# TheoCoombes/ClipCap

Measured on AMD Instinct MI355X. Metric: train samples/sec (512-d prefix, 40-tok caption), higher is better.
Workload: dtype bf16; 1 GPU; BASELINE configs[1]: TransformerMapper(8L,P=L=10,H=8)+frozen GPT-2-small; per_gpu_batch=256, global_batch=256, encoder_dim=512, train_language_model=False, parallelism=dp1

## Files before the change

clipcap_amd/csrc/attention.hip:

```cpp
#include "kernels.h"

namespace CC_NS {

__device__ __forceinline__ void load_head_rows(float* dst, int hdp, const act_t* src, size_t ld, int S, int hd) {
    const int c8n = hd >> 3;
    for (int idx = threadIdx.x; idx < S * c8n; idx += blockDim.x) {
        const int r = idx / c8n, c = idx % c8n;
        float f[8];
        act_ld8(src + (size_t)r * ld + c * 8, f);
        float* d = dst + r * hdp + c * 8;
        *reinterpret_cast<float4*>(d) = make_float4(f[0], f[1], f[2], f[3]);
        *reinterpret_cast<float4*>(d + 4) = make_float4(f[4], f[5], f[6], f[7]);
    }
}

template <auto Kernel, class... Args>
static void attn_launch(dim3 grid, dim3 block, size_t sh, hipStream_t st, const Args&... args) {
    if (sh > 64 * 1024) (void)hipFuncSetAttribute((const void*)Kernel, hipFuncAttributeMaxDynamicSharedMemorySize, (int)sh);
    hipLaunchKernelGGL(Kernel, grid, block, sh, st, args...);
}
#define ATTN_LADDER(LAUNCH) { if (drop.thresh) { LAUNCH(true, true); } else if (causal) { LAUNCH(true, false); } else { LAUNCH(false, false); } }

__device__ __forceinline__ unsigned attn_drop_idx(int b, int H, int h, int S, int q, int k) { return ((unsigned)(b * H + h) * S + q) * S + k; }
template <bool CAUSAL>
// ... 579 lines not shown
        }
        float mx = -INFINITY;
#pragma unroll
        for (int r = 0; r < 16; r++) {
            const int kr = kb * 32 + c_row(r, half);
            const bool ok = kr < S && (!CAUSAL || kr <= q);
            s[r] = ok ? s[r] * scale : -INFINITY;
            mx = fmaxf(mx, s[r]);
        }
        mx = fmaxf(mx, __shfl_xor(mx, 32, 64));
        const float m_new = fmaxf(m, mx);
        const float alpha = (m == -INFINITY) ? 0.f : __expf(m - m_new);
        float p[16], ps = 0.f;
#pragma unroll
        for (int r = 0; r < 16; r++) {
            p[r] = (m_new == -INFINITY) ? 0.f : __expf(s[r] - m_new);
            ps += p[r];
        }
        ps += __shfl_xor(ps, 32, 64);
        l = l * alpha + ps;
        m = m_new;
#pragma unroll
        for (int nb = 0; nb < NB; nb++)
#pragma unroll
            for (int r = 0; r < 16; r++) o[nb][r] *= alpha;
        if (DROP) {
            const unsigned rowbase = attn_drop_idx(b, H, h, S, min(q, S - 1), 0);
#pragma unroll
            for (int r = 0; r < 16; r++) p[r] *= drop_mul(drop, rowbase + min(kb * 32 + c_row(r, half), S - 1));
        }
        op16x8 pf[2];
#pragma unroll
        for (int t = 0; t < 2; t++) pf[t] = pack_frag(p + t * 8);
#pragma unroll
        for (int t = 0; t < 2; t++)
#pragma unroll
            for (int nb = 0; nb < NB; nb++) o[nb] = CC_MFMA_32x32x16(frag_tr<HD>(vs, nb, t, lane), pf[t], o[nb]);
#pragma unroll
        for (int kk = 0; kk < KK; kk++) kq[kk] = kn[kk];
#pragma unroll
        for (int c = 0; c < HD / 16; c++) vq[c] = vn[c];
    }
    if (q < S) {
        const float inv = l > 0.f ? 1.f / l : 0.f;
        op16_t* orow = out + ((size_t)b * S + q) * D + h * HD;
        store_acc_row<NB, true>(orow, o, half, inv);
        if (half == 0 && lse_out) lse_out[((size_t)b * H + h) * S + q] = m + __logf(l);
    }
}

template <int HD>
static int attn_fwd_mfma_launch(const op16_t* qkv, int B, int S, int H, bool causal, op16_t* out, float* lse, hipStream_t st, Drop drop) {
    const int items = B * H * ((S + 31) / 32);
    const float scale = 1.0f / sqrtf((float)HD);
    if (drop.thresh && !causal) return CC_ERR_SHAPE;
#define CC_L(C, DR) attn_launch<k_attn_fwd_mfma<HD, C, DR>>(dim3((items + 3) / 4), dim3(256), 0, st, qkv, B, S, H, scale, out, lse, drop)
    ATTN_LADDER(CC_L)
#undef CC_L
    return hipGetLastError() == hipSuccess ? CC_OK : CC_ERR_LAUNCH;
}


template <int HD, bool CAUSAL, bool DROP = false>
__global__ __launch_bounds__(256, HD == 64 ? 2 : 1) void k_attn_bwd_dkv(const op16_t* __restrict__ qkv, const op16_t* __restrict__ dout,
                                                      const float* __restrict__ lse, const float* __restrict__ delta, int B, int S, int H,
                                                      float scale, op16_t* __restrict__ dqkv, Drop drop = Drop()) {
    constexpr int KK = HD / 16, NB = HD / 32;
    __shared__ __attribute__((aligned(16))) op16_t qsm[4][32 * AttLd<HD>::v];
    __shared__ __attribute__((aligned(16))) op16_t dsm[4][32 * AttLd<HD>::v];
    __shared__ __attribute__((aligned(16))) float ldsm[4][64];
    const int lane = threadIdx.x & 63, wave = threadIdx.x >> 6;
    const int nblk = (S + 31) >> 5;
    const int item = blockIdx.x * 4 + wave;
    if (item >= B * H * nblk) return;
    const int j = item % nblk, h = (item / nblk) % H, b = item / (nblk * H);
    const int D = H * HD;
    const size_t rs = (size_t)3 * D;
    const op16_t* base = qkv + (size_t)b * S * rs + h * HD;
    const op16_t* dbase = dout + (size_t)b * S * D + h * HD;
    const float* lrow = lse + ((size_t)b * H + h) * S;
    const float* drow = delta + ((size_t)b * H + h) * S;
    const int half = lane >> 5, key = j * 32 + (lane & 31);
    op16x8 kf[KK], vf[KK];
#pragma unroll
    for (int kk = 0; kk < KK; kk++) {
        kf[kk] = load_frag(base + D + (size_t)min(key, S - 1) * rs + kk * 16 + half * 8, key < S);
        vf[kk] = load_frag(base + 2 * D + (size_t)min(key, S - 1) * rs + kk * 16 + half * 8, key < S);
    }
    f32x16 dk[NB], dv[NB];
#pragma unroll
    for (int nb = 0; nb < NB; nb++)
#pragma unroll
        for (int r = 0; r < 16; r++) { dk[nb][r] = 0.f; dv[nb][r] = 0.f; }
    const int i0 = CAUSAL ? j : 0;
    op16x8 qf[KK], df[KK];
    {
        const int qa = i0 * 32 + (lane & 31);
#pragma unroll
        for (int kk = 0; kk < KK; kk++) {
            qf[kk] = load_frag(base + (size_t)min(qa, S - 1) * rs + kk * 16 + half * 8, qa < S);
            df[kk] = load_frag(dbase + (size_t)min(qa, S - 1) * D + kk * 16 + half * 8, qa < S);
        }
    }
    for (int i = i0; i < nblk; i++) {
        op16x8 qn[KK], dn[KK];
        {
            const int qa = (i + 1) * 32 + (lane & 31);
#pragma unroll
            for (int kk = 0; kk < KK; kk++) {
                qn[kk] = load_frag(base + (size_t)min(qa, S - 1) * rs + kk * 16 + half * 8, qa < S);
                dn[kk] = load_frag(dbase + (size_t)min(qa, S - 1) * D + kk * 16 + half * 8, qa < S);
            }
        }
        f32x16 s, dp;
#pragma unroll
        for (int r = 0; r < 16; r++) { s[r] = 0.f; dp[r] = 0.f; }
#pragma unroll
        for (int kk = 0; kk < KK; kk++) {
            s = CC_MFMA_32x32x16(qf[kk], kf[kk], s);
            dp = CC_MFMA_32x32x16(df[kk], vf[kk], dp);
            *reinterpret_cast<op16x8*>(qsm[wave] + (lane & 31) * AttLd<HD>::v + kk * 16 + half * 8) = qf[kk];
            *reinterpret_cast<op16x8*>(dsm[wave] + (lane & 31) * AttLd<HD>::v + kk * 16 + half * 8) = df[kk];
        }
        {
            const int qq = min(i * 32 + (lane & 31), S - 1);
            ldsm[wave][lane] = half ? drow[qq] : lrow[qq];
        }
        float lq[16], dq_[16];
#pragma unroll
        for (int g4 = 0; g4 < 4; g4++) {
            const float4 a = *reinterpret_cast<const float4*>(&ldsm[wave][4 * half + 8 * g4]);
            const float4 b = *reinterpret_cast<const float4*>(&ldsm[wave][32 + 4 * half + 8 * g4]);
            lq[g4 * 4 + 0] = a.x; lq[g4 * 4 + 1] = a.y; lq[g4 * 4 + 2] = a.z; lq[g4 * 4 + 3] = a.w;
            dq_[g4 * 4 + 0] = b.x; dq_[g4 * 4 + 1] = b.y; dq_[g4 * 4 + 2] = b.z; dq_[g4 * 4 + 3] = b.w;
        }
        float p[16], ds[16];
#pragma unroll
        for (int r = 0; r < 16; r++) {
            const int qr = i * 32 + c_row(r, half);
            const bool ok = attn_live<CAUSAL>(qr, key, S);
            p[r] = ok ? __expf(s[r] * scale - lq[r]) : 0.f;
            if (DROP) {
                const float mk = drop_mul(drop, attn_drop_idx(b, H, h, S, min(qr, S - 1), min(key, S - 1)));
                ds[r] = p[r] * (mk * dp[r] - dq_[r]) * scale;
                p[r] *= mk;
            } else {
                ds[r] = p[r] * (dp[r] - dq_[r]) * scale;
            }
        }
        const op16x8 pf[2] = {pack_frag(p), pack_frag(p + 8)};
        const op16x8 dsf[2] = {pack_frag(ds), pack_frag(ds + 8)};
#pragma unroll
        for (int t = 0; t < 2; t++)
#pragma unroll
            for (int nb = 0; nb < NB; nb++) {
                dv[nb] = CC_MFMA_32x32x16(frag_tr<HD>(dsm[wave], nb, t, lane), pf[t], dv[nb]);
                dk[nb] = CC_MFMA_32x32x16(frag_tr<HD>(qsm[wave], nb, t, lane), dsf[t], dk[nb]);
            }
#pragma unroll
        for (int kk = 0; kk < KK; kk++) { qf[kk] = qn[kk]; df[kk] = dn[kk]; }
    }
    if (key < S) {
        op16_t* orow = dqkv + ((size_t)b * S + key) * rs + h * HD;
#pragma unroll
        for (int nb = 0; nb < NB; nb++)
#pragma unroll
            for (int g = 0; g < 4; g++) {
                const int d0 = nb * 32 + 8 * g + 4 * half;
                *reinterpret_cast<uint2*>(orow + D + d0) =
                    make_uint2(pack2op(dk[nb][g * 4 + 0], dk[nb][g * 4 + 1]), pack2op(dk[nb][g * 4 + 2], dk[nb][g * 4 + 3]));
                *reinterpret_cast<uint2*>(orow + 2 * D + d0) =
                    make_uint2(pack2op(dv[nb][g * 4 + 0], dv[nb][g * 4 + 1]), pack2op(dv[nb][g * 4 + 2], dv[nb][g * 4 + 3]));
            }
    }
}

template <int HD, bool CAUSAL, bool DROP = false>
__global__ __launch_bounds__(256, HD == 64 ? 3 : (HD == 96 ? 2 : 1)) void k_attn_bwd_dq(const op16_t* __restrict__ qkv, const op16_t* __restrict__ dout, const op16_t* __restrict__ o,
                                                     const float* __restrict__ lse, float* __restrict__ delta, int B, int S, int H,
                                                     float scale, op16_t* __restrict__ dqkv, Drop drop = Drop()) {
    constexpr int KK = HD / 16, NB = HD / 32;
    __shared__ __attribute__((aligned(16))) op16_t ksm[4][32 * AttLd<HD>::v];
    const int lane = threadIdx.x & 63, wave = threadIdx.x >> 6;
    const int nblk = (S + 31) >> 5;
    const int item = blockIdx.x * 4 + wave;
    if (item >= B * H * nblk) return;
    const int i = item % nblk, h = (item / nblk) % H, b = item / (nblk * H);
    const int D = H * HD;
    const size_t rs = (size_t)3 * D;
    const op16_t* base = qkv + (size_t)b * S * rs + h * HD;
    const op16_t* dbase = dout + (size_t)b * S * D + h * HD;
    const int half = lane >> 5, q = i * 32 + (lane & 31);
    const float my_lse = q < S ? lse[((size_t)b * H + h) * S + q] : 0.f;
    op16x8 qf[KK], dof[KK];
    float my_delta = 0.f;
#pragma unroll
    for (int kk = 0; kk < KK; kk++) {
        qf[kk] = load_frag(base + (size_t)min(q, S - 1) * rs + kk * 16 + half * 8, q < S);
        dof[kk] = load_frag(dbase + (size_t)min(q, S - 1) * D + kk * 16 + half * 8, q < S);
        const op16x8 of = load_frag(o + ((size_t)b * S + min(q, S - 1)) * D + h * HD + kk * 16 + half * 8, q < S);
        float x[8], y[8];
        unpack8(__builtin_bit_cast(uint4, dof[kk]), x);
        unpack8(__builtin_bit_cast(uint4, of), y);
#pragma unroll
        for (int e = 0; e < 8; e++) my_delta += x[e] * y[e];
    }
    my_delta += __shfl_xor(my_delta, 32, 64);
    if (half == 0 && q < S) delta[((size_t)b * H + h) * S + q] = my_delta;
    f32x16 dq[NB];
#pragma unroll
    for (int nb = 0; nb < NB; nb++)
#pragma unroll
        for (int r = 0; r < 16; r++) dq[nb][r] = 0.f;
    const int jend = CAUSAL ? i + 1 : nblk;
    op16x8 kf[KK], vf[KK];
    {
        const int key = lane & 31;
#pragma unroll
        for (int kk = 0; kk < KK; kk++) {
            kf[kk] = load_frag(base + D + (size_t)min(key, S - 1) * rs + kk * 16 + half * 8, key < S);
            vf[kk] = load_frag(base + 2 * D + (size_t)min(key, S - 1) * rs + kk * 16 + half * 8, key < S);
        }
    }
    for (int j = 0; j < jend; j++) {
        op16x8 kn[KK], vn[KK];
        {
            const int key = (j + 1) * 32 + (lane & 31);
#pragma unroll
            for (int kk = 0; kk < KK; kk++) {
                kn[kk] = load_frag(base + D + (size_t)min(key, S - 1) * rs + kk * 16 + half * 8, key < S);
                vn[kk] = load_frag(base + 2 * D + (size_t)min(key, S - 1) * rs + kk * 16 + half * 8, key < S);
            }
        }
        f32x16 st, dpt;
#pragma unroll
        for (int r = 0; r < 16; r++) { st[r] = 0.f; dpt[r] = 0.f; }
#pragma unroll
        for (int kk = 0; kk < KK; kk++) {
            st = CC_MFMA_32x32x16(kf[kk], qf[kk], st);
            dpt = CC_MFMA_32x32x16(vf[kk], dof[kk], dpt);
            *reinterpret_cast<op16x8*>(ksm[wave] + (lane & 31) * AttLd<HD>::v + kk * 16 + half * 8) = kf[kk];
        }
        float ds[16];
#pragma unroll
        for (int r = 0; r < 16; r++) {
            const int kr = j * 32 + c_row(r, half);
            const bool ok = kr < S && q < S && (!CAUSAL || kr <= q);
            const float p = ok ? __expf(st[r] * scale - my_lse) : 0.f;
            const float mk = DROP ? drop_mul(drop, attn_drop_idx(b, H, h, S, min(q, S - 1), min(kr, S - 1))) : 1.0f;
            ds[r] = p * (mk * dpt[r] - my_delta) * scale;
        }
        const op16x8 dsf[2] = {pack_frag(ds), pack_frag(ds + 8)};
#pragma unroll
        for (int t = 0; t < 2; t++)
#pragma unroll
            for (int nb = 0; nb < NB; nb++)
                dq[nb] = CC_MFMA_32x32x16(frag_tr<HD>(ksm[wave], nb, t, lane), dsf[t], dq[nb]);
#pragma unroll
        for (int kk = 0; kk < KK; kk++) { kf[kk] = kn[kk]; vf[kk] = vn[kk]; }
    }
    if (q < S) {
        op16_t* orow = dqkv + ((size_t)b * S + q) * rs + h * HD;
        store_acc_row<NB>(orow, dq, half);
    }
}

#ifndef CC_ATTN_FUSED_OCC
#define CC_ATTN_FUSED_OCC 2
#endif
template <int LD, int ROWS = 32>
__device__ __forceinline__ op16x8 frag_tr_ld(const op16_t* blk, int nb, int t, int lane) {
    typedef __attribute__((ext_vector_type(4))) short s16x4_t;
    typedef __attribute__((address_space(3))) s16x4_t* lp_t;
    const int half = lane >> 5, j = lane & 15, dsub = (lane >> 4) & 1;
    const int r0 = 16 * t + 4 * half + (j >> 2);
    const op16_t* col = blk + nb * 32 + 16 * dsub + 4 * (j & 3);
    const op16_t* p = col + (ROWS < 32 ? min(r0, ROWS - 1) : r0) * LD;
    const op16_t* ph = col + (ROWS < 32 ? min(r0 + 8, ROWS - 1) : r0 + 8) * LD;
    const s16x4_t lo = __builtin_amdgcn_ds_read_tr16_b64_v4i16((lp_t)p);
    const s16x4_t hi = __builtin_amdgcn_ds_read_tr16_b64_v4i16((lp_t)ph);
    typedef __attribute__((ext_vector_type(8))) short s16x8_t;
    const s16x8_t v = {lo[0], lo[1], lo[2], lo[3], hi[0], hi[1], hi[2], hi[3]};
    return __builtin_bit_cast(op16x8, v);
}

template <int HD>
__device__ __forceinline__ void attn_store_tile(op16_t* T, const f32x16 (&acc)[HD / 32], op16_t* gblock, size_t gstride, int rows_left, int lane) {
    constexpr int LD = AttLd<HD>::v, C8 = HD / 8;
    const int half = lane >> 5, l31 = lane & 31;
#pragma unroll
    for (int nb = 0; nb < HD / 32; nb++)
#pragma unroll
        for (int g = 0; g < 4; g++)
            *reinterpret_cast<uint2*>(T + l31 * LD + nb * 32 + 8 * g + 4 * half) =
                make_uint2(pack2op(acc[nb][g * 4 + 0], acc[nb][g * 4 + 1]), pack2op(acc[nb][g * 4 + 2], acc[nb][g * 4 + 3]));
#pragma unroll
    for (int it = 0; it < C8 / 2; it++) {
        const int idx = lane + 64 * it, row = idx / C8, chunk = idx % C8;
        const uint4 v = *reinterpret_cast<const uint4*>(T + row * LD + chunk * 8);
        if (row < rows_left) *reinterpret_cast<uint4*>(gblock + (size_t)row * gstride + chunk * 8) = v;
    }
}

template <int HD, bool CAUSAL, bool DROP, int NBLK, int OCC, int DR = 32>
__global__ __launch_bounds__(256, OCC) void k_attn_bwd_fused(const op16_t* __restrict__ qkv, const op16_t* __restrict__ dout, const op16_t* __restrict__ o,
                                                             const float* __restrict__ lse, int B, int S, int H, float scale,
                                                             op16_t* __restrict__ dqkv, Drop drop = Drop()) {
    constexpr int KK = HD / 16, NB = HD / 32, LD = AttLd<HD>::v;
    constexpr bool SPARE = LD >= HD + 32;
    constexpr int LT = SPARE ? LD : 32;
    __shared__ __attribute__((aligned(16))) op16_t ksm[4][32 * LD];
    __shared__ __attribute__((aligned(16))) op16_t qsm[4][32 * LD];
    __shared__ __attribute__((aligned(16))) op16_t dsm[4][32 * LD];
    static_assert(DR == 32 || (!SPARE && NBLK == 1), "the short dS^T tile is for the single-block form with its own tile");
    __shared__ __attribute__((aligned(16))) op16_t dtx[SPARE ? 1 : 4][SPARE ? 8 : DR * 32];
    __shared__ __attribute__((aligned(16))) float ldsm[4][NBLK][64];
    const int lane = threadIdx.x & 63, wave = threadIdx.x >> 6;
    const int item = blockIdx.x * 4 + wave;
    if (item >= B * H) return;
    const int h = item % H, b = item / H;
    const int D = H * HD;
    const size_t rs = (size_t)3 * D;
    const op16_t* base = qkv + (size_t)b * S * rs + h * HD;
    const op16_t* dbase = dout + (size_t)b * S * D + h * HD;
    const op16_t* obase = o + (size_t)b * S * D + h * HD;
    const float* lrow = lse + ((size_t)b * H + h) * S;
    const int half = lane >> 5, l31 = lane & 31;
    const int coff = half * 8;
    op16_t* dtm = SPARE ? ksm[wave] + HD : dtx[SPARE ? 0 : wave];

    op16x8 qf[KK], dof[KK], kf[KK], vf[KK];
    auto load_q = [&](int i) {
        const int q = i * 32 + l31, qc = min(q, S - 1);
#pragma unroll
        for (int kk = 0; kk < KK; kk++) {
            qf[kk] = load_frag(base + (size_t)qc * rs + kk * 16 + coff, q < S);
            dof[kk] = load_frag(dbase + (size_t)qc * D + kk * 16 + coff, q < S);
        }
    };
    auto load_k = [&](int j) {
        const int key = j * 32 + l31, kc = min(key, S - 1);
#pragma unroll
        for (int kk = 0; kk < KK; kk++) {
            kf[kk] = load_frag(base + D + (size_t)kc * rs + kk * 16 + coff, key < S);
            vf[kk] = load_frag(base + 2 * D + (size_t)kc * rs + kk * 16 + coff, key < S);
        }
    };
    load_k(0);
    load_q(0);
#pragma unroll
    for (int i = 0; i < NBLK; i++) {
        const int q = i * 32 + l31, qc = min(q, S - 1);
        float acc = 0.f;
#pragma unroll
        for (int kk = 0; kk < KK; kk++) {
            const op16x8 df = load_frag(dbase + (size_t)qc * D + kk * 16 + coff, q < S);
            const op16x8 of = load_frag(obase + (size_t)qc * D + kk * 16 + coff, q < S);
            float x[8], y[8];
            unpack8(__builtin_bit_cast(uint4, df), x);
            unpack8(__builtin_bit_cast(uint4, of), y);
#pragma unroll
            for (int e = 0; e < 8; e++) acc += x[e] * y[e];
        }
        acc += __shfl_xor(acc, 32, 64);
        ldsm[wave][i][lane] = half ? acc : lrow[qc];
    }
    f32x16 dq[NBLK][NB];

#pragma unroll
    for (int j = 0; j < NBLK; j++) {
        const int key = j * 32 + l31;
#pragma unroll
        for (int kk = 0; kk < KK; kk++) *reinterpret_cast<op16x8*>(ksm[wave] + l31 * LD + kk * 16 + coff) = kf[kk];
        f32x16 dk[NB], dv[NB];
#pragma unroll
        for (int nb = 0; nb < NB; nb++)
#pragma unroll
            for (int r = 0; r < 16; r++) { dk[nb][r] = 0.f; dv[nb][r] = 0.f; }
#pragma unroll
        for (int i = 0; i < NBLK; i++) {
            if (CAUSAL && i < j) continue;
            const int ifirst = CAUSAL ? j : 0;
            if (!(j > 0 && i == ifirst && i == NBLK - 1)) {
#pragma unroll
                for (int kk = 0; kk < KK; kk++) {
                    *reinterpret_cast<op16x8*>(qsm[wave] + l31 * LD + kk * 16 + coff) = qf[kk];
                    *reinterpret_cast<op16x8*>(dsm[wave] + l31 * LD + kk * 16 + coff) = dof[kk];
                }
            }
            f32x16 s, dp;
#pragma unroll
            for (int r = 0; r < 16; r++) { s[r] = 0.f; dp[r] = 0.f; }
#pragma unroll
            for (int kk = 0; kk < KK; kk++) {
                s = CC_MFMA_32x32x16(qf[kk], kf[kk], s);
                dp = CC_MFMA_32x32x16(dof[kk], vf[kk], dp);
            }
            if (i + 1 < NBLK) {
                load_q(i + 1);
            } else if (j + 1 < NBLK) {
                const int ni = CAUSAL ? j + 1 : 0;
                if (ni != i) load_q(ni);
                load_k(j + 1);
            }
            if (j == 0) {
#pragma unroll
                for (int nb = 0; nb < NB; nb++)
#pragma unroll
                    for (int r = 0; r < 16; r++) dq[i][nb][r] = 0.f;
            }
            float p[16], ds[16];
#pragma unroll
            for (int g4 = 0; g4 < 4; g4++) {
                const float4 lq = *reinterpret_cast<const float4*>(&ldsm[wave][i][4 * half + 8 * g4]);
                const float4 dl = *reinterpret_cast<const float4*>(&ldsm[wave][i][32 + 4 * half + 8 * g4]);
                const float lqa[4] = {lq.x, lq.y, lq.z, lq.w}, dla[4] = {dl.x, dl.y, dl.z, dl.w};
#pragma unroll
                for (int e = 0; e < 4; e++) {
                    const int r = g4 * 4 + e;
                    const int qr = i * 32 + c_row(r, half);
                    const bool ok = qr < S && key < S && (!CAUSAL || key <= qr);
                    p[r] = ok ? __expf(s[r] * scale - lqa[e]) : 0.f;
                    if (DROP) {
                        const float mk = drop_mul(drop, attn_drop_idx(b, H, h, S, min(qr, S - 1), min(key, S - 1)));
                        ds[r] = p[r] * (mk * dp[r] - dla[e]) * scale;
                        p[r] *= mk;
                    } else {
                        ds[r] = p[r] * (dp[r] - dla[e]) * scale;
                    }
                }
            }
            const op16x8 pf[2] = {pack_frag(p), pack_frag(p + 8)};
            const op16x8 dsf[2] = {pack_frag(ds), pack_frag(ds + 8)};
            if (DR == 32 || l31 < DR) {
#pragma unroll
                for (int t = 0; t < 2; t++) {
                    const uint4 w = __builtin_bit_cast(uint4, dsf[t]);
                    *reinterpret_cast<uint2*>(dtm + l31 * LT + 16 * t + 4 * half) = make_uint2(w.x, w.y);
                    *reinterpret_cast<uint2*>(dtm + l31 * LT + 16 * t + 8 + 4 * half) = make_uint2(w.z, w.w);
                }
            }
#pragma unroll
            for (int t = 0; t < 2; t++)
#pragma unroll
                for (int nb = 0; nb < NB; nb++) {
                    dv[nb] = CC_MFMA_32x32x16(frag_tr<HD>(dsm[wave], nb, t, lane), pf[t], dv[nb]);
                    dk[nb] = CC_MFMA_32x32x16(frag_tr<HD>(qsm[wave], nb, t, lane), dsf[t], dk[nb]);
                }
#pragma unroll
            for (int t = 0; t < 2; t++) {
                const op16x8 dst = frag_tr_ld<LT, DR>(dtm, 0, t, lane);
#pragma unroll
                for (int nb = 0; nb < NB; nb++) dq[i][nb] = CC_MFMA_32x32x16(frag_tr<HD>(ksm[wave], nb, t, lane), dst, dq[i][nb]);
            }
            if (j == (CAUSAL ? i : NBLK - 1)) {
                attn_store_tile<HD>(qsm[wave], dq[i], dqkv + ((size_t)b * S + i * 32) * rs + h * HD, rs, S - i * 32, lane);
            }
        }
        {
            op16_t* gblk = dqkv + ((size_t)b * S + j * 32) * rs + h * HD;
            attn_store_tile<HD>(ksm[wave], dk, gblk + D, rs, S - j * 32, lane);
            attn_store_tile<HD>(ksm[wave], dv, gblk + 2 * D, rs, S - j * 32, lane);
        }
    }
}

template <int HD, int NBLK>
static void attn_bwd_fused_launch(const op16_t* qkv, const op16_t* dout, const op16_t* o, const float* lse, int B, int S, int H, bool causal,
                                  op16_t* dqkv, hipStream_t st, Drop drop, float scale) {
    constexpr int OCC = CC_ATTN_FUSED_OCC;
    const dim3 grid((B * H + 3) / 4), blk(256);
#define CC_L(C, DR) attn_launch<k_attn_bwd_fused<HD, C, DR, NBLK, (C && HD == 64 ? OCC : 1)>>(grid, blk, 0, st, qkv, dout, o, lse, B, S, H, scale, dqkv, drop)
    if (drop.thresh || causal) ATTN_LADDER(CC_L)
    else {
        if constexpr (HD == 96 && NBLK == 1) {
            static const bool short_on = []() { const char* e = cc_lab_env("CC_ATTN_BWD_SHORT"); return !e || atoi(e) != 0; }();
            if (S <= 24 && short_on) {
                attn_launch<k_attn_bwd_fused<HD, false, false, NBLK, 2, 24>>(grid, blk, 0, st, qkv, dout, o, lse, B, S, H, scale, dqkv, drop);
                return;
            }
        }
        CC_L(false, false);
    }
#undef CC_L
}

template <int HD>
static int attn_bwd_mfma_launch(const op16_t* qkv, const op16_t* dout, const op16_t* o, const float* lse, float* delta, int B, int S, int H,
                                bool causal, op16_t* dqkv, hipStream_t st, Drop drop) {
    const int items = B * H * ((S + 31) / 32);
    const float scale = 1.0f / sqrtf((float)HD);
    if (drop.thresh && !causal) return CC_ERR_SHAPE;
    static const int fused = []() { const char* e = cc_lab_env("CC_ATTN_BWD_FUSED"); return e ? atoi(e) : 1; }();
    if (fused && S <= 32) {
        attn_bwd_fused_launch<HD, 1>(qkv, dout, o, lse, B, S, H, causal, dqkv, st, drop, scale);
        return hipGetLastError() == hipSuccess ? CC_OK : CC_ERR_LAUNCH;
    }
    if constexpr (HD < 128) {
        if (fused && S <= 64) {
            attn_bwd_fused_launch<HD, 2>(qkv, dout, o, lse, B, S, H, causal, dqkv, st, drop, scale);
            return hipGetLastError() == hipSuccess ? CC_OK : CC_ERR_LAUNCH;
        }
    }
#define CC_L(C, DR)                                                                                                                         \
    attn_launch<k_attn_bwd_dq<HD, C, DR>>(dim3((items + 3) / 4), dim3(256), 0, st, qkv, dout, o, lse, delta, B, S, H, scale, dqkv, drop); \
    attn_launch<k_attn_bwd_dkv<HD, C, DR>>(dim3((items + 3) / 4), dim3(256), 0, st, qkv, dout, lse, delta, B, S, H, scale, dqkv, drop)
    ATTN_LADDER(CC_L)
#undef CC_L
    return hipGetLastError() == hipSuccess ? CC_OK : CC_ERR_LAUNCH;
}

#endif

static size_t attn_fwd_lds(int S, int hd) { return ((size_t)3 * S * (hd + 4) + (size_t)S * (S + 1)) * 4; }
static size_t attn_bwd_lds(int S, int hd) {
    if (S < 32) return ((size_t)4 * S * (hd + 4) + (size_t)2 * S * (S + 1)) * 4;
    const size_t S4 = (S + 3) & ~3;
    return ((size_t)4 * S4 * (hd + 4) + (size_t)2 * S4 * (S4 + 4)) * 4;
}

__global__ __launch_bounds__(256) void k_attn_probs(const act_t* __restrict__ qkv, int B, int S, int H, int hd, float scale,
                                                    float* __restrict__ out) {
    const int wave = blockIdx.x * 4 + (threadIdx.x >> 6), lane = threadIdx.x & 63;
    if (wave >= B * H * S) return;
    const int n = wave % S, h = (wave / S) % H, b = wave / (S * H);
    const int D = H * hd;
    const act_t* q = qkv + ((size_t)b * S + n) * 3 * D + h * hd;
    float mx = -INFINITY;
    for (int m0 = 0; m0 < S; m0 += 64) {
        const int m = m0 + lane;
        float sc = -INFINITY;
        if (m < S) {
            const act_t* k = qkv + ((size_t)b * S + m) * 3 * D + D + h * hd;
            float acc = 0.f;
            for (int d = 0; d < hd; d++) acc += act2f(q[d]) * act2f(k[d]);
            sc = acc * scale;
            out[(((size_t)b * S + n) * S + m) * H + h] = sc;
        }
        mx = fmaxf(mx, wave_max(sc));
    }
    float sum = 0.f;
    for (int m = lane; m < S; m += 64) sum += __expf(out[(((size_t)b * S + n) * S + m) * H + h] - mx);
    sum = wave_sum(sum);
    for (int m = lane; m < S; m += 64) {
        float* o = out + (((size_t)b * S + n) * S + m) * H + h;
        *o = __expf(*o - mx) / sum;
    }
}
int attn_probs(const act_t* qkv, int B, int S, int H, int hd, float* out, hipStream_t st) {
    const int waves = B * H * S;
    if (waves <= 0) return CC_OK;
    hipLaunchKernelGGL(k_attn_probs, dim3((waves + 3) / 4), dim3(256), 0, st, qkv, B, S, H, hd, 1.0f / sqrtf((float)hd), out);
    return CC_OK;
}

#if CC_OP == 2
__device__ __forceinline__ float row_dot(const float* a, const float* b, int hd) {
    float s0 = 0.f, s1 = 0.f;
    for (int d = 0; d < hd; d += 8) {
        const float4 x0 = *reinterpret_cast<const float4*>(a + d), y0 = *reinterpret_cast<const float4*>(b + d);
        const float4 x1 = *reinterpret_cast<const float4*>(a + d + 4), y1 = *reinterpret_cast<const float4*>(b + d + 4);
        s0 += x0.x * y0.x + x0.y * y0.y + x0.z * y0.z + x0.w * y0.w;
        s1 += x1.x * y1.x + x1.y * y1.y + x1.z * y1.z + x1.w * y1.w;
    }
    return s0 + s1;
}
template <bool CAUSAL>
__global__ __launch_bounds__(256) void k_attn_fwd_rows(const float* __restrict__ qkv, int B, int S, int H, int hd, float scale, float* __restrict__ out,
                                                       float* __restrict__ lse) {
    extern __shared__ float rsm[];
    const int lane = threadIdx.x & 63, wave = threadIdx.x >> 6;
    const int item = blockIdx.x * 4 + wave;
    if (item >= B * H * S) return;
    const int i = item % S, h = (item / S) % H, b = item / (S * H);
    const int D = H * hd;
    const size_t rs = (size_t)3 * D;
    const float* base = qkv + (size_t)b * S * rs + h * hd;
    const float* q = base + (size_t)i * rs;
    float* p = rsm + wave * S;
    const int nk = CAUSAL ? i + 1 : S;
    float m = -INFINITY;
    for (int j = lane; j < nk; j += 64) {
        const float sc = row_dot(q, base + D + (size_t)j * rs, hd) * scale;
        p[j] = sc;
        m = fmaxf(m, sc);
    }
    m = wave_max(m);
    float sum = 0.f;
    for (int j = lane; j < nk; j += 64) {
        const float e = __expf(p[j] - m);
        p[j] = e;
        sum += e;
    }
    sum = wave_sum(sum);
    const float inv = 1.f / sum;
    for (int d = lane; d < hd; d += 64) {
        float o = 0.f;
        const float* v = base + 2 * D + d;
        for (int j = 0; j < nk; j++) o += p[j] * v[(size_t)j * rs];
        out[((size_t)b * S + i) * D + h * hd + d] = o * inv;
    }
    if (lane == 0 && lse) lse[((size_t)b * H + h) * S + i] = m + __logf(sum);
}
template <bool CAUSAL>
__global__ __launch_bounds__(256) void k_attn_bwd_rows_dq(const float* __restrict__ qkv, const float* __restrict__ dout, const float* __restrict__ o,
                                                          const float* __restrict__ lse, float* __restrict__ delta, int B, int S, int H, int hd,
                                                          float scale, float* __restrict__ dqkv) {
    extern __shared__ float rsm[];
    const int lane = threadIdx.x & 63, wave = threadIdx.x >> 6;
    const int item = blockIdx.x * 4 + wave;
    if (item >= B * H * S) return;
    const int i = item % S, h = (item / S) % H, b = item / (S * H);
    const int D = H * hd;
    const size_t rs = (size_t)3 * D;
    const float* base = qkv + (size_t)b * S * rs + h * hd;
    const float* q = base + (size_t)i * rs;
    const float* dor = dout + ((size_t)b * S + i) * D + h * hd;
    const float* orow = o + ((size_t)b * S + i) * D + h * hd;
    float* ds = rsm + wave * S;
    float dl = 0.f;
    for (int d = lane; d < hd; d += 64) dl += dor[d] * orow[d];
    dl = wave_sum(dl);
    const float l = lse[((size_t)b * H + h) * S + i];
    if (lane == 0) delta[((size_t)b * H + h) * S + i] = dl;
    const int nk = CAUSAL ? i + 1 : S;
    for (int j = lane; j < nk; j += 64) {
        const float pj = __expf(row_dot(q, base + D + (size_t)j * rs, hd) * scale - l);
        const float dp = row_dot(dor, base + 2 * D + (size_t)j * rs, hd);
        ds[j] = pj * (dp - dl) * scale;
    }
    for (int d = lane; d < hd; d += 64) {
        float acc = 0.f;
        const float* k = base + D + d;
        for (int j = 0; j < nk; j++) acc += ds[j] * k[(size_t)j * rs];
        dqkv[((size_t)b * S + i) * rs + h * hd + d] = acc;
    }
}
template <bool CAUSAL>
__global__ __launch_bounds__(256) void k_attn_bwd_rows_dkv(const float* __restrict__ qkv, const float* __restrict__ dout, const float* __restrict__ lse,
                                                           const float* __restrict__ delta, int B, int S, int H, int hd, float scale,
                                                           float* __restrict__ dqkv) {
    extern __shared__ float rsm[];
    const int lane = threadIdx.x & 63, wave = threadIdx.x >> 6;
    const int item = blockIdx.x * 4 + wave;
    if (item >= B * H * S) return;
    const int j = item % S, h = (item / S) % H, b = item / (S * H);
    const int D = H * hd;
    const size_t rs = (size_t)3 * D;
    const float* base = qkv + (size_t)b * S * rs + h * hd;
    const float* k = base + D + (size_t)j * rs;
    const float* v = base + 2 * D + (size_t)j * rs;
    const float* dbase = dout + (size_t)b * S * D + h * hd;
    const float* lrow = lse + ((size_t)b * H + h) * S;
    const float* drow = delta + ((size_t)b * H + h) * S;
    float* pp = rsm + wave * 2 * S;
    float* ds = pp + S;
    const int i0 = CAUSAL ? j : 0;
    for (int i = i0 + lane; i < S; i += 64) {
        const float pij = __expf(row_dot(base + (size_t)i * rs, k, hd) * scale - lrow[i]);
        const float dp = row_dot(dbase + (size_t)i * D, v, hd);
        pp[i] = pij;
        ds[i] = pij * (dp - drow[i]) * scale;
    }
    for (int d = lane; d < hd; d += 64) {
        float dk = 0.f, dv = 0.f;
        for (int i = i0; i < S; i++) {
            dk += ds[i] * base[(size_t)i * rs + d];
            dv += pp[i] * dbase[(size_t)i * D + d];
        }
        float* orow = dqkv + ((size_t)b * S + j) * rs + h * hd + d;
        orow[D] = dk;
        orow[2 * D] = dv;
    }
}
static int attn_fwd_rows(const float* qkv, int B, int S, int H, int hd, bool causal, float* out, float* lse, float scale, hipStream_t st) {
    if (S > 2048) return CC_ERR_SHAPE;
    const int items = B * H * S;
    const size_t sh = (size_t)4 * S * sizeof(float);
    if (causal) hipLaunchKernelGGL(k_attn_fwd_rows<true>, dim3((items + 3) / 4), dim3(256), sh, st, qkv, B, S, H, hd, scale, out, lse);
    else hipLaunchKernelGGL(k_attn_fwd_rows<false>, dim3((items + 3) / 4), dim3(256), sh, st, qkv, B, S, H, hd, scale, out, lse);
    return hipGetLastError() == hipSuccess ? CC_OK : CC_ERR_LAUNCH;
}
static int attn_bwd_rows(const float* qkv, const float* dout, const float* o, const float* lse, float* delta, int B, int S, int H, int hd,
                         bool causal, float* dqkv, float scale, hipStream_t st) {
    if (S > 2048) return CC_ERR_SHAPE;
    const int items = B * H * S;
    const dim3 gr((items + 3) / 4), bl(256);
    const size_t sh1 = (size_t)4 * S * sizeof(float), sh2 = 2 * sh1;
    if (causal) {
        hipLaunchKernelGGL(k_attn_bwd_rows_dq<true>, gr, bl, sh1, st, qkv, dout, o, lse, delta, B, S, H, hd, scale, dqkv);
        hipLaunchKernelGGL(k_attn_bwd_rows_dkv<true>, gr, bl, sh2, st, qkv, dout, lse, delta, B, S, H, hd, scale, dqkv);
    } else {
        hipLaunchKernelGGL(k_attn_bwd_rows_dq<false>, gr, bl, sh1, st, qkv, dout, o, lse, delta, B, S, H, hd, scale, dqkv);
        hipLaunchKernelGGL(k_attn_bwd_rows_dkv<false>, gr, bl, sh2, st, qkv, dout, lse, delta, B, S, H, hd, scale, dqkv);
    }
    return hipGetLastError() == hipSuccess ? CC_OK : CC_ERR_LAUNCH;
}

#ifdef CC_EXPERIMENTS
typedef float v16f __attribute__((ext_vector_type(16)));
#define CC_MFMA_F32(a, b, c) __builtin_amdgcn_mfma_f32_32x32x2f32(a, b, c, 0, 0, 0)

__device__ __forceinline__ void load_head_rows_pad(float* dst, int hdp, const float* src, size_t ld, int S, int RP, int hd) {
    const int c4n = hd >> 2;
    for (int idx = threadIdx.x; idx < RP * c4n; idx += blockDim.x) {
        const int r = idx / c4n, c = idx % c4n;
        const float4 v = r < S ? *reinterpret_cast<const float4*>(src + (size_t)r * ld + c * 4) : make_float4(0, 0, 0, 0);
        *reinterpret_cast<float4*>(dst + r * hdp + c * 4) = v;
    }
}
__device__ __forceinline__ void mm_rows_rows(v16f& acc, const float* X, int r0, const float* Y, int c0, int hdp, int hd, int lane) {
    const float* xa = X + (r0 + (lane & 31)) * hdp + 4 * (lane >> 5);
    const float* yb = Y + (c0 + (lane & 31)) * hdp + 4 * (lane >> 5);
    for (int d8 = 0; d8 < hd; d8 += 8) {
        const float4 a = *reinterpret_cast<const float4*>(xa + d8), b = *reinterpret_cast<const float4*>(yb + d8);
        acc = CC_MFMA_F32(a.x, b.x, acc);
        acc = CC_MFMA_F32(a.y, b.y, acc);
        acc = CC_MFMA_F32(a.z, b.z, acc);
        acc = CC_MFMA_F32(a.w, b.w, acc);
    }
}

template <bool CAUSAL, bool DROP>
__global__ __launch_bounds__(256) void k_attn_fwd_f32mfma(const float* __restrict__ qkv, int S, int H, int hd, float scale, float* __restrict__ out,
                                                          float* __restrict__ lse, Drop drop) {
    extern __shared__ __attribute__((aligned(16))) float sm[];
    const int D = H * hd, hdp = hd + 4, NT = (S + 31) >> 5, RP = NT * 32, Sp = RP + 4;
    float* Qs = sm;
    float* Ks = Qs + RP * hdp;
    float* Vs = Ks + RP * hdp;
    float* Ps = Vs + RP * hdp;
    const int b = blockIdx.x / H, h = blockIdx.x % H;
    const float* base = qkv + (size_t)b * S * 3 * D + h * hd;
    load_head_rows_pad(Qs, hdp, base, 3 * D, S, RP, hd);
    load_head_rows_pad(Ks, hdp, base + D, 3 * D, S, RP, hd);
    load_head_rows_pad(Vs, hdp, base + 2 * D, 3 * D, S, RP, hd);
    __syncthreads();
    const int lane = threadIdx.x & 63, wave = threadIdx.x >> 6, lr = lane & 31, lh = lane >> 5;
    for (int t = wave; t < NT * NT; t += 4) {
        const int ti = t / NT, tj = t - ti * NT;
        v16f acc;
        acc_zero(acc);
        if (!(CAUSAL && tj > ti)) mm_rows_rows(acc, Qs, ti * 32, Ks, tj * 32, hdp, hd, lane);
        const int j = tj * 32 + lr;
#pragma unroll
        for (int r = 0; r < 16; r++) {
            const int i = ti * 32 + 8 * (r >> 2) + 4 * lh + (r & 3);
            Ps[i * Sp + j] = (j < S && !(CAUSAL && j > i)) ? acc[r] * scale : -INFINITY;
        }
    }
    __syncthreads();
    for (int i = wave; i < S; i += 4) {
        float m = -INFINITY;
        for (int j = lane; j < RP; j += 64) m = fmaxf(m, Ps[i * Sp + j]);
        m = wave_max(m);
        float sum = 0.f;
        for (int j = lane; j < RP; j += 64) {
            const float e = __expf(Ps[i * Sp + j] - m);
            Ps[i * Sp + j] = e;
            sum += e;
        }
        sum = wave_sum(sum);
        const float inv = 1.f / sum;
        for (int j = lane; j < RP; j += 64) Ps[i * Sp + j] *= inv;
        if (lane == 0 && lse) lse[((size_t)b * H + h) * S + i] = m + __logf(sum);
    }
    for (int i = S + wave; i < RP; i += 4)
        for (int j = lane; j < RP; j += 64) Ps[i * Sp + j] = 0.f;
    __syncthreads();
    const int nd = hd >> 5;
    for (int t = wave; t < NT * nd; t += 4) {
        const int ti = t / nd, td = t - ti * nd;
        v16f acc;
        acc_zero(acc);
        const int jmax = CAUSAL ? (ti + 1) * 32 : RP;
        const int i = ti * 32 + lr;
        const float* pa = Ps + i * Sp + 4 * lh;
        const float* vb = Vs + 4 * lh * hdp + td * 32 + lr;
        for (int j8 = 0; j8 < jmax; j8 += 8) {
            float4 a = *reinterpret_cast<const float4*>(pa + j8);
            if (DROP) {
                const unsigned e0 = attn_drop_idx(b, H, h, S, i, j8 + 4 * lh);
                a.x *= drop_mul(drop, e0); a.y *= drop_mul(drop, e0 + 1); a.z *= drop_mul(drop, e0 + 2); a.w *= drop_mul(drop, e0 + 3);
            }
            const float* v = vb + j8 * hdp;
            acc = CC_MFMA_F32(a.x, v[0], acc);
            acc = CC_MFMA_F32(a.y, v[hdp], acc);
            acc = CC_MFMA_F32(a.z, v[2 * hdp], acc);
            acc = CC_MFMA_F32(a.w, v[3 * hdp], acc);
        }
#pragma unroll
        for (int r = 0; r < 16; r++) {
            const int io = ti * 32 + 8 * (r >> 2) + 4 * lh + (r & 3);
            if (io < S) out[((size_t)b * S + io) * D + h * hd + td * 32 + lr] = acc[r];
        }
    }
}

template <bool CAUSAL, bool DROP>
__global__ __launch_bounds__(256) void k_attn_bwd_f32mfma(const float* __restrict__ qkv, const float* __restrict__ dout, const float* __restrict__ lse,
                                                          int S, int H, int hd, float scale, float* __restrict__ dqkv, Drop drop) {
    extern __shared__ __attribute__((aligned(16))) float sm[];
    const int D = H * hd, hdp = hd + 4, NT = (S + 31) >> 5, RP = NT * 32, Sp = RP + 4;
// ... 473 lines not shown
```

Baseline: 22230 samples/s.

## Make fused attention backward persistent with cross-item prefetch of next head

Measured after the change: 22330 samples/s (median of 6 runs). No clear change (+0.4%).

```diff
diff --git a/clipcap_amd/csrc/attention.hip b/clipcap_amd/csrc/attention.hip
--- a/clipcap_amd/csrc/attention.hip
+++ b/clipcap_amd/csrc/attention.hip
@@ -905,6 +905,7 @@
     }
 }
 
+template <int HD, bool DROP, int NBLK, int OCC> struct AttBwdWalk { static constexpr bool v = !(OCC == 2 && (HD > 64 || (DROP && NBLK == 2))); };
 template <int HD, bool CAUSAL, bool DROP, int NBLK, int OCC, int DR = 32>
 __global__ __launch_bounds__(256, OCC) void k_attn_bwd_fused(const op16_t* __restrict__ qkv, const op16_t* __restrict__ dout, const op16_t* __restrict__ o,
                                                              const float* __restrict__ lse, int B, int S, int H, float scale,
@@ -919,27 +920,36 @@
     __shared__ __attribute__((aligned(16))) op16_t dtx[SPARE ? 1 : 4][SPARE ? 8 : DR * 32];
     __shared__ __attribute__((aligned(16))) float ldsm[4][NBLK][64];
     const int lane = threadIdx.x & 63, wave = threadIdx.x >> 6;
-    const int item = blockIdx.x * 4 + wave;
-    if (item >= B * H) return;
-    const int h = item % H, b = item / H;
+    constexpr bool WALK = AttBwdWalk<HD, DROP, NBLK, OCC>::v;
+    const int items = B * H, stride = gridDim.x * 4;
+    int item = __builtin_amdgcn_readfirstlane(blockIdx.x * 4 + wave);
+    if (item >= items) return;
     const int D = H * HD;
     const size_t rs = (size_t)3 * D;
-    const op16_t* base = qkv + (size_t)b * S * rs + h * HD;
-    const op16_t* dbase = dout + (size_t)b * S * D + h * HD;
-    const op16_t* obase = o + (size_t)b * S * D + h * HD;
-    const float* lrow = lse + ((size_t)b * H + h) * S;
     const int half = lane >> 5, l31 = lane & 31;
     const int coff = half * 8;
     op16_t* dtm = SPARE ? ksm[wave] + HD : dtx[SPARE ? 0 : wave];
 
-    op16x8 qf[KK], dof[KK], kf[KK], vf[KK];
-    auto load_q = [&](int i) {
+    const op16_t *base, *dbase, *obase;
+    const float* lrow;
+    auto point = [&](int it) {
+        const int h = it % H, b = it / H;
+        base = qkv + (size_t)b * S * rs + h * HD;
+        dbase = dout + (size_t)b * S * D + h * HD;
+        obase = o + (size_t)b * S * D + h * HD;
+        lrow = lse + ((size_t)b * H + h) * S;
+    };
+    op16x8 qf[KK], dof[KK], of[KK], kf[KK], vf[KK];
+    float lv = 0.f;
+    auto load_q = [&](int i, bool wo) {
         const int q = i * 32 + l31, qc = min(q, S - 1);
 #pragma unroll
         for (int kk = 0; kk < KK; kk++) {
             qf[kk] = load_frag(base + (size_t)qc * rs + kk * 16 + coff, q < S);
             dof[kk] = load_frag(dbase + (size_t)qc * D + kk * 16 + coff, q < S);
-        }
+            if (wo) of[kk] = load_frag(obase + (size_t)qc * D + kk * 16 + coff, q < S);
+        }
+        if (wo) lv = lrow[qc];
     };
     auto load_k = [&](int j) {
         const int key = j * 32 + l31, kc = min(key, S - 1);
@@ -949,25 +959,14 @@
             vf[kk] = load_frag(base + 2 * D + (size_t)kc * rs + kk * 16 + coff, key < S);
         }
     };
+    point(item);
     load_k(0);
-    load_q(0);
-#pragma unroll
-    for (int i = 0; i < NBLK; i++) {
-        const int q = i * 32 + l31, qc = min(q, S - 1);
-        float acc = 0.f;
-#pragma unroll
-        for (int kk = 0; kk < KK; kk++) {
-            const op16x8 df = load_frag(dbase + (size_t)qc * D + kk * 16 + coff, q < S);
-            const op16x8 of = load_frag(obase + (size_t)qc * D + kk * 16 + coff, q < S);
-            float x[8], y[8];
-            unpack8(__builtin_bit_cast(uint4, df), x);
-            unpack8(__builtin_bit_cast(uint4, of), y);
-#pragma unroll
-            for (int e = 0; e < 8; e++) acc += x[e] * y[e];
-        }
-        acc += __shfl_xor(acc, 32, 64);
-        ldsm[wave][i][lane] = half ? acc : lrow[qc];
-    }
+    load_q(0, true);
+    for (;;) {
+    const int h = item % H, b = item / H;
+    op16_t* gbase = dqkv + (size_t)b * S * rs + h * HD;
+    const bool more = WALK && item + stride < items;
+    const int nitem = more ? item + stride : item;
     f32x16 dq[NBLK][NB];
 
 #pragma unroll
@@ -984,6 +983,19 @@
         for (int i = 0; i < NBLK; i++) {
             if (CAUSAL && i < j) continue;
             const int ifirst = CAUSAL ? j : 0;
+            if (j == 0) {
+                float acc = 0.f;
+#pragma unroll
+                for (int kk = 0; kk < KK; kk++) {
+                    float x[8], y[8];
+                    unpack8(__builtin_bit_cast(uint4, dof[kk]), x);
+                    unpack8(__builtin_bit_cast(uint4, of[kk]), y);
+#pragma unroll
+                    for (int e = 0; e < 8; e++) acc += x[e] * y[e];
+                }
+                acc += __shfl_xor(acc, 32, 64);
+                ldsm[wave][i][lane] = half ? acc : lv;
+            }
             if (!(j > 0 && i == ifirst && i == NBLK - 1)) {
 #pragma unroll
                 for (int kk = 0; kk < KK; kk++) {
@@ -1000,11 +1012,15 @@
                 dp = CC_MFMA_32x32x16(dof[kk], vf[kk], dp);
             }
             if (i + 1 < NBLK) {
-                load_q(i + 1);
+                load_q(i + 1, j == 0);
             } else if (j + 1 < NBLK) {
                 const int ni = CAUSAL ? j + 1 : 0;
-                if (ni != i) load_q(ni);
+                if (ni != i) load_q(ni, false);
                 load_k(j + 1);
+            } else if (more) {
+                point(nitem);
+                load_k(0);
+                load_q(0, true);
             }
             if (j == 0) {
 #pragma unroll
@@ -1057,29 +1073,47 @@
                 for (int nb = 0; nb < NB; nb++) dq[i][nb] = CC_MFMA_32x32x16(frag_tr<HD>(ksm[wave], nb, t, lane), dst, dq[i][nb]);
             }
             if (j == (CAUSAL ? i : NBLK - 1)) {
-                attn_store_tile<HD>(qsm[wave], dq[i], dqkv + ((size_t)b * S + i * 32) * rs + h * HD, rs, S - i * 32, lane);
+                attn_store_tile<HD>(qsm[wave], dq[i], gbase + (size_t)i * 32 * rs, rs, S - i * 32, lane);
             }
         }
         {
-            op16_t* gblk = dqkv + ((size_t)b * S + j * 32) * rs + h * HD;
+            op16_t* gblk = gbase + (size_t)j * 32 * rs;
             attn_store_tile<HD>(ksm[wave], dk, gblk + D, rs, S - j * 32, lane);
             attn_store_tile<HD>(ksm[wave], dv, gblk + 2 * D, rs, S - j * 32, lane);
         }
     }
-}
-
+    if (!more) break;
+    item = nitem;
+    }
+}
+
+static int attn_ncu() {
+    static int ncu = 0;
+    if (!ncu) {
+        int dev = 0;
+        hipDeviceProp_t pr;
+        if (hipGetDevice(&dev) != hipSuccess || hipGetDeviceProperties(&pr, dev) != hipSuccess) return 0;
+        ncu = pr.multiProcessorCount;
+    }
+    return ncu;
+}
 template <int HD, int NBLK>
 static void attn_bwd_fused_launch(const op16_t* qkv, const op16_t* dout, const op16_t* o, const float* lse, int B, int S, int H, bool causal,
-                                  op16_t* dqkv, hipStream_t st, Drop drop, float scale) {
+                                  op16_t* dqkv, hipStream_t st, Drop drop, float scale, int ncu) {
     constexpr int OCC = CC_ATTN_FUSED_OCC;
-    const dim3 grid((B * H + 3) / 4), blk(256);
-#define CC_L(C, DR) attn_launch<k_attn_bwd_fused<HD, C, DR, NBLK, (C && HD == 64 ? OCC : 1)>>(grid, blk, 0, st, qkv, dout, o, lse, B, S, H, scale, dqkv, drop)
+    const int wgs = (B * H + 3) / 4;
+    const dim3 blk(256);
+    auto grid_of = [&](bool walk, int occ) { return dim3(walk ? min(wgs, ncu * occ) : wgs); };
+#define CC_L(C, DR)                                                                                                                \
+    attn_launch<k_attn_bwd_fused<HD, C, DR, NBLK, (C && HD == 64 ? OCC : 1)>>(grid_of(AttBwdWalk<HD, DR, NBLK, (C && HD == 64 ? OCC : 1)>::v, \
+                                                                                      (C && HD == 64 ? OCC : 1)),                 \
+                                                                              blk, 0, st, qkv, dout, o, lse, B, S, H, scale, dqkv, drop)
     if (drop.thresh || causal) ATTN_LADDER(CC_L)
     else {
         if constexpr (HD == 96 && NBLK == 1) {
             static const bool short_on = []() { const char* e = cc_lab_env("CC_ATTN_BWD_SHORT"); return !e || atoi(e) != 0; }();
             if (S <= 24 && short_on) {
-                attn_launch<k_attn_bwd_fused<HD, false, false, NBLK, 2, 24>>(grid, blk, 0, st, qkv, dout, o, lse, B, S, H, scale, dqkv, drop);
+                attn_launch<k_attn_bwd_fused<HD, false, false, NBLK, 2, 24>>(grid_of(AttBwdWalk<HD, false, NBLK, 2>::v, 2), blk, 0, st, qkv, dout, o, lse, B, S, H, scale, dqkv, drop);
                 return;
             }
         }
@@ -1095,13 +1129,15 @@
     const float scale = 1.0f / sqrtf((float)HD);
     if (drop.thresh && !causal) return CC_ERR_SHAPE;
     static const int fused = []() { const char* e = cc_lab_env("CC_ATTN_BWD_FUSED"); return e ? atoi(e) : 1; }();
+    const int ncu = attn_ncu();
+    if (!ncu) return CC_ERR_STATE;
     if (fused && S <= 32) {
-        attn_bwd_fused_launch<HD, 1>(qkv, dout, o, lse, B, S, H, causal, dqkv, st, drop, scale);
+        attn_bwd_fused_launch<HD, 1>(qkv, dout, o, lse, B, S, H, causal, dqkv, st, drop, scale, ncu);
         return hipGetLastError() == hipSuccess ? CC_OK : CC_ERR_LAUNCH;
     }
     if constexpr (HD < 128) {
         if (fused && S <= 64) {
-            attn_bwd_fused_launch<HD, 2>(qkv, dout, o, lse, B, S, H, causal, dqkv, st, drop, scale);
+            attn_bwd_fused_launch<HD, 2>(qkv, dout, o, lse, B, S, H, causal, dqkv, st, drop, scale, ncu);
             return hipGetLastError() == hipSuccess ? CC_OK : CC_ERR_LAUNCH;
         }
     }
```
